# GabrieleCocco/CLFaceDetection

Measured on AMD Instinct MI355X. Metric: candidate windows/sec, 1080p, haarcascade_frontalface_alt, higher is better.
Workload: dtype u32 gathers + f32 stage sums; 1 GPU; BASELINE config 3: 64x1920x1080 8-bit frames per step in the whole job (noise/smooth/blocks mix; sharded by whole frames over 1 GPU), haarcascade_frontalface_alt, scaleFactor 1.1f, raw candidates, frames resident in HBM; frames_on_rank_0=64, windows_per_frame=6290352, parallelism=single GPU, device=AMD Radeon Graphics (gfx950:sramecc+:xnack-), 256 CUs, pipeline=vj_stream, two batches in flight

## Files before the change

clfacedetection_amd/csrc/vj_env.cpp:

```cpp
#include "vj_internal.hpp"
#include "vj_device.hpp"

#include <hip/hip_runtime_api.h>

#include <algorithm>
#include <climits>
#include <cmath>
#include <cstdint>
#include <cstdio>
#include <cstdlib>
#include <cstring>
#include <map>
#include <memory>
#include <string>
#include <tuple>

#include "vj_env_internal.hpp"

using namespace vj;

namespace vj {

static uint32_t f2u(float f) {
    uint32_t u;
// ... 743 lines not shown
        HIP_TRY(hipStreamSynchronize(e->stream));
        if (e->stream2) HIP_TRY(hipStreamSynchronize(e->stream2));
        while ((int)e->plans.size() >= std::max(2, e->plan_cache_max)) {
            auto lru = e->plans.begin();
            for (auto i = e->plans.begin(); i != e->plans.end(); ++i)
                if (i->second->last_used < lru->second->last_used) lru = i;
            lru->second->release_device();
            e->plans.erase(lru);
        }
    }
    auto pl = std::make_unique<Plan>();
    TileThresholds th{e->tile_min_windows, e->tile_accept_windows, e->tile_max_dwords_per_window};
    if (small == 2) th = TileThresholds{64, 64, 8000};
    else if (small == 1) th = TileThresholds{256, 256, 2000};
    else if (small == 3) th = TileThresholds{std::min(384, th.min_windows), std::min(384, th.accept_windows), th.max_dwords_per_window};
    int rc = build_plan(e, *c, W, H, p, pl.get(), split, th, one_pass);
    if (rc) {
        pl->release_device();
        return rc;
    }
    pl->last_used = ++e->plan_tick;
    *out = pl.get();
    e->plans[key] = std::move(pl);
    return VJ_OK;
}

int Lane::create() {
    for (auto& x : ev) HIP_TRY(hipEventCreate(&x));
    for (auto& x : pass_ev) HIP_TRY(hipEventCreate(&x));
    for (auto& x : launch_ev) HIP_TRY(hipEventCreate(&x));
    HIP_TRY(hipEventCreateWithFlags(&upload_done, hipEventDisableTiming));
    HIP_TRY(hipEventCreateWithFlags(&integral_done, hipEventDisableTiming));
    HIP_TRY(hipEventCreateWithFlags(&done, hipEventDisableTiming));
    h_pinned_bytes = (size_t)1 << 20;
    HIP_TRY(hipHostMalloc(&h_pinned, h_pinned_bytes, hipHostMallocDefault));
    return VJ_OK;
}

void Lane::destroy() {
    for (DevBuf* b : {&d_gray, &d_counts, &d_det}) b->release();
    if (h_pinned) (void)hipHostFree(h_pinned);
    if (h_stage) (void)hipHostFree(h_stage);
    h_pinned = h_stage = nullptr;
    for (auto& x : ev) if (x) (void)hipEventDestroy(x);
    for (auto& x : pass_ev) if (x) (void)hipEventDestroy(x);
    for (auto& x : launch_ev) if (x) (void)hipEventDestroy(x);
    for (hipEvent_t* x : {&upload_done, &integral_done, &done}) if (*x) (void)hipEventDestroy(*x);
}

int ensure_image_buffers(vj_env* e, int W, int H, int frames, bool need_gray, int channels, Lane* lane) {
    if (!lane) lane = &e->lane0;
    const size_t fe = frame_elems_for(W, H);
    const uint32_t n_bands = ((uint32_t)H + BAND_ROWS - 1) / BAND_ROWS;
    const uint32_t band_pitch = ((uint32_t)W + 3u) & ~3u;
    int rc;
    const size_t sum_bytes = fe * 4 * (size_t)frames, sq_bytes = fe * 8 * (size_t)frames;
    const bool grow = sum_bytes > e->d_sum.cap || sq_bytes > e->d_sqsum.cap;
    if ((rc = e->d_sum.ensure(sum_bytes))) return rc;
    if ((rc = e->d_sqsum.ensure(sq_bytes))) return rc;
    (void)grow;
    if (need_gray) {
        const size_t gstride = ((size_t)W * (size_t)channels + 3) & ~(size_t)3;
        if ((rc = lane->d_gray.ensure(gstride * (size_t)H * (size_t)frames))) return rc;
    }
    const size_t band_elems = (size_t)frames * n_bands * band_pitch;
    if ((rc = e->d_band_sum.ensure(band_elems * 4))) return rc;
    if ((rc = e->d_band_sq.ensure(band_elems * 4))) return rc;
    if ((rc = e->d_band_sqp.ensure(band_elems * 8))) return rc;
    return VJ_OK;
}

int enqueue_integral(vj_env* e, const uint8_t* d_gray, size_t frame_bytes, int stride, int W, int H, int frames,
                     int channels) {
    IntegralArgs ia;
    memset(&ia, 0, sizeof(ia));
    ia.channels = (uint32_t)channels;
    ia.gray = d_gray;
    ia.gray_frame_bytes = frame_bytes;
    ia.gray_stride = (uint32_t)stride;
    ia.width = (uint32_t)W;
    ia.height = (uint32_t)H;
    ia.n_frames = (uint32_t)frames;
    ia.n_bands = ((uint32_t)H + BAND_ROWS - 1) / BAND_ROWS;
    ia.band_pitch = ((uint32_t)W + 3u) & ~3u;
    ia.band_sum = (uint32_t*)e->d_band_sum.p;
    ia.band_sq = (uint32_t*)e->d_band_sq.p;
    ia.band_sq_prefix = (uint64_t*)e->d_band_sqp.p;
    ia.sum = (uint32_t*)e->d_sum.p;
    ia.sqsum = (uint64_t*)e->d_sqsum.p;
    ia.frame_elems = frame_elems_for(W, H);
    ia.rows_mode = (uint32_t)e->integral_rows_mode;
    const size_t used = (size_t)(W + 1) * (size_t)(H + 1);
    const bool zeroed = e->slack_w == W && e->slack_h == H && e->slack_frames >= frames && e->slack_sum == e->d_sum.p &&
                        e->slack_sq == e->d_sqsum.p;
    for (int f = 0; f < frames && !zeroed; ++f) {
        HIP_TRY(hipMemsetAsync((uint32_t*)e->d_sum.p + (size_t)f * ia.frame_elems + used, 0,
                               (ia.frame_elems - used) * 4, e->stream));
        HIP_TRY(hipMemsetAsync((uint64_t*)e->d_sqsum.p + (size_t)f * ia.frame_elems + used, 0,
                               (ia.frame_elems - used) * 8, e->stream));
    }
    if (!zeroed) {
        e->slack_w = W;
        e->slack_h = H;
        e->slack_frames = frames;
        e->slack_sum = e->d_sum.p;
        e->slack_sq = e->d_sqsum.p;
    }
    int hrc = launch_integral(ia, e->stream);
    if (hrc) {
        set_error("integral launch failed: %s", hipGetErrorString((hipError_t)hrc));
        return VJ_ERR_HIP;
    }
    return VJ_OK;
}

int enqueue_tilted(vj_env* e, const uint8_t* d_gray, size_t frame_bytes, int stride, int W, int H, int frames, int channels) {
    const uint32_t fe = frame_elems_for(W, H);
    int rc;
    if ((rc = e->d_tilted.ensure((size_t)fe * 4u * (size_t)frames))) return rc;
    HIP_TRY(hipMemsetAsync(e->d_tilted.p, 0, (size_t)fe * 4u * (size_t)frames, e->stream));
    TiltedArgs ta;
    memset(&ta, 0, sizeof(ta));
    ta.gray = d_gray;
    ta.gray_frame_bytes = frame_bytes;
    ta.gray_stride = (uint32_t)stride;
    ta.channels = (uint32_t)channels;
    ta.width = (uint32_t)W;
    ta.height = (uint32_t)H;
    ta.n_frames = (uint32_t)frames;
    ta.frame_elems = fe;
    ta.tilted = (uint32_t*)e->d_tilted.p;
    const size_t n_bands = ((size_t)H + 7u) / 8u;
    if ((rc = e->d_tilt_diag.ensure((size_t)frames * n_bands * 2u * (size_t)(W + H) * 4u))) return rc;
    if ((rc = e->d_tilt_col.ensure((size_t)frames * n_bands * (size_t)(W + 1) * 4u))) return rc;
    const int hrc = launch_tilted_bands(ta, (uint32_t*)e->d_tilt_diag.p, (uint32_t*)e->d_tilt_col.p, e->stream);
    if (hrc) {
        set_error("tilted integral launch failed (width %d): %s", W, hipGetErrorString((hipError_t)hrc));
        return hrc == (int)hipErrorInvalidValue ? VJ_ERR_LIMIT : VJ_ERR_HIP;
    }
    return VJ_OK;
}
// ... 88 lines not shown
                for (int y = 0; y < H; ++y) memcpy(st + (size_t)y * gstride, src + (size_t)y * src_stride, row_bytes);
                src = st;
                src_stride = gstride;
            }
        }
        HIP_TRY(hipMemcpy2DAsync(dst, gstride, src, src_stride, row_bytes, (size_t)H,
                                 frames[i].on_device ? hipMemcpyDeviceToDevice : hipMemcpyHostToDevice, cs));
    }
    *d_ptr = (const uint8_t*)lane->d_gray.p;
    *stride = (int)gstride;
    *frame_bytes = gstride * (size_t)H;
    return VJ_OK;
}

struct RawDet {
    int frame;
    uint32_t slot, x, y;
};

struct CountsLayout {
    static constexpr size_t q_counts = (size_t)MAX_SCALES * Q_PARTS;
    static constexpr size_t stage_off_u32 = MAX_PASSES * q_counts + 2;
    static constexpr size_t roi_off_u32 = stage_off_u32 + (size_t)(1 + VJ_MAX_LAUNCHES) * VJ_MAX_STAGES * 2;
    static constexpr size_t q2_off_u32 = roi_off_u32 + 8 + (size_t)VJ_MAX_STAGES * 2;
    static constexpr size_t bytes = (q2_off_u32 + MAX_PASSES * q_counts) * sizeof(uint32_t);
};

static int enqueue_prepare(vj_env* e, Lane* L, Plan* pl, const vj_image* frames, int nf, int W, int H, bool fixed_queue_layout,
                           hipStream_t copy_stream) {
    int rc;
    const int channels = image_channels(frames[0]);
    if ((rc = ensure_image_buffers(e, W, H, nf, true, channels, L))) return rc;
    uint64_t q_entries = 0;
    if (!fixed_queue_layout) {
        if ((rc = layout_queues(pl, nf, &q_entries))) return rc;
        const size_t n_pass = pl->pass_bounds.size() - 1;
        for (size_t ps = 1; ps < n_pass; ++ps)
            if ((rc = e->d_q[ps].ensure(std::max<uint64_t>(q_entries, 1) * sizeof(QEntry)))) return rc;
    }
    if ((rc = L->d_counts.ensure(CountsLayout::bytes))) return rc;
    if (L->det_cap == 0) {
        L->det_cap = e->det_cap_init;
        if ((rc = L->d_det.ensure((size_t)L->det_cap * sizeof(DetEntry)))) return rc;
    }
    const uint8_t* d_gray;
    size_t gray_frame_bytes;
    int gray_stride;
    if ((rc = stage_frames(e, frames, nf, W, H, &d_gray, &gray_frame_bytes, &gray_stride, L, copy_stream))) return rc;
    if (copy_stream) {
        HIP_TRY(hipEventRecord(L->upload_done, copy_stream));
        HIP_TRY(hipStreamWaitEvent(e->stream, L->upload_done, 0));
    }
    L->src_gray = d_gray;
    L->src_frame_bytes = gray_frame_bytes;
    L->src_stride = gray_stride;
    L->src_channels = channels;
    HIP_TRY(hipEventRecord(L->ev[0], e->stream));
    if ((rc = enqueue_integral(e, d_gray, gray_frame_bytes, gray_stride, W, H, nf, channels))) return rc;
    HIP_TRY(hipEventRecord(L->ev[1], e->stream));
    HIP_TRY(hipEventRecord(L->integral_done, e->stream));
    L->nf = nf;
    return VJ_OK;
}

static int enqueue_cascade(vj_env* e, Lane* L, Plan* pl, int W, int , const vj_params& p) {
    int rc;
    const int nf = L->nf;
    const size_t n_pass = pl->pass_bounds.size() - 1;
    const size_t counts_bytes = CountsLayout::bytes;
    constexpr size_t q_counts = CountsLayout::q_counts;
    uint32_t* d_qcount[MAX_PASSES];
    for (int ps = 0; ps < MAX_PASSES; ++ps) d_qcount[ps] = (uint32_t*)L->d_counts.p + ps * q_counts;
    uint32_t* d_qcount2[MAX_PASSES];
    for (int ps = 0; ps < MAX_PASSES; ++ps) d_qcount2[ps] = (uint32_t*)L->d_counts.p + CountsLayout::q2_off_u32 + ps * q_counts;
    uint32_t* d_det_count = (uint32_t*)L->d_counts.p + MAX_PASSES * q_counts;
    unsigned long long* d_stage_entered = (unsigned long long*)((uint32_t*)L->d_counts.p + CountsLayout::stage_off_u32);
    const bool count = (p.flags & VJ_FLAG_COUNTERS) != 0;
    const int n_blocks = std::max(1, e->n_cu * e->blocks_per_cu);
    {
        HIP_TRY(hipMemsetAsync(L->d_counts.p, 0, counts_bytes, e->stream));
        HIP_TRY(hipEventRecord(L->ev[2], e->stream));
        CascadeArgs ca;
        memset(&ca, 0, sizeof(ca));
        ca.sum = (const uint32_t*)e->d_sum.p;
        ca.sqsum = (const uint64_t*)e->d_sqsum.p;
        ca.table = (const uint32_t*)pl->d_table.p;
        ca.scales = (const ScaleDev*)pl->d_scales.p;
        ca.stages = (const StageDev*)pl->d_stages.p;
        ca.units = (const UnitDev*)pl->d_units.p;
        ca.n_units = (uint32_t)pl->units.size();
        ca.tile_units = (const UnitDev*)pl->d_tile_units.p;
        ca.n_tile_units = (uint32_t)pl->tile_units.size();
        ca.n_frames = (uint32_t)nf;
        ca.n_scales = (uint32_t)pl->scales.size();
        ca.frame_elems = pl->frame_elems;
        ca.sum_bytes = (uint32_t)((uint64_t)pl->frame_elems * 4u * (uint64_t)nf);
        ca.stride = (uint32_t)W + 1u;
        ca.gather_waves = (uint32_t)e->gather_waves_for(nf, pl->general);
        ca.total_waves = (uint32_t)n_blocks * ca.gather_waves;
        ca.det = (DetEntry*)L->d_det.p;
        ca.det_count = d_det_count;
        ca.det_cap = L->det_cap;
        ca.signed_mean = (p.flags & VJ_FLAG_SIGNED_MEAN) ? 1u : 0u;
        ca.stage_entered = d_stage_entered;
        ca.tree_ctr = d_stage_entered;
        ca.n_pass = (uint32_t)n_pass;
        for (size_t ps = 0; ps <= n_pass; ++ps) ca.pass_begin[ps] = pl->pass_bounds[ps];
        for (size_t ps = 1; ps < n_pass; ++ps) {
            ca.q_pass[ps] = (QEntry*)e->d_q[ps].p;
            ca.q_pass_count[ps] = d_qcount[ps];
        }
        ca.tile_end = pl->general ? pl->general_prefix : (uint32_t)e->tile_end;
        ca.tile_min_lanes = (uint32_t)e->tile_min_lanes;
        ca.tile_repack_mask = e->tile_repack_mask;
        ca.tile_sp_begin = (!pl->general && (pl->wave_tail || pl->tree2)) ? (uint32_t)e->tile_sp_begin : 0xffffffffu;
        ca.tree2 = pl->tree2 ? 1u : 0u;
        ca.identity_order = pl->general ? 0u : 1u;
        ca.n_seg = e->tile_segments ? pl->tile_n_seg : 0u;
        for (int k = 0; k < 4; ++k) ca.seg_end[k] = pl->tile_seg_end[k];
        ca.seg_chain = pl->tile_seg_chain;
        ca.sp_blocks = (const SpBlock*)pl->d_sp_blocks.p;
        ca.n_sp_blocks = pl->n_sp_blocks;
        ca.tile_ws_min = pl->wave_tail ? (uint32_t)e->tile_ws_min : 0u;
        ca.tile_ws_max = (uint32_t)std::min(e->tile_ws_max, (int)TILE_WS_MAX_WINDOWS);
        ca.pos_mode = pl->pos_mode;
        ca.pos_tab = (const uint32_t*)pl->d_pos_tab.p;
        ca.gather_pairs = e->pairs_for(nf);
        ca.sp_tail_max = (uint32_t)std::max(0, std::min(e->sp_tail_max, 48));
        ca.max_stage_nodes = pl->max_stage_nodes;
        if (pl->skip_mode && pl->n_skip_units) {
            if ((rc = e->d_skip_bits.ensure((size_t)pl->skip_frame_words * 8u * (size_t)nf))) return rc;
            ca.skip_bits = (unsigned long long*)e->d_skip_bits.p;
            ca.skip_frame_words = pl->skip_frame_words;
            ca.skip_units = (const UnitDev*)pl->d_skip_units.p;
            ca.n_skip_units = pl->n_skip_units;
            ca.skip_segs = (const UnitDev*)pl->d_skip_segs.p;
            ca.n_skip_segs = pl->n_skip_segs;
            const int hrc = launch_skip_bitmap(ca, pl->trees, std::max(1, e->n_cu * 4), e->stream);
            if (hrc) {
                set_error("skip bitmap launch failed: %s", hipGetErrorString((hipError_t)hrc));
                return VJ_ERR_HIP;
            }
        }
        int launches = 0;
        std::vector<vj_launch>& linfo = L->linfo;
        linfo.clear();
        auto begin_launch = [&](int kind, int cls, uint32_t sb, uint32_t se, uint32_t lds, hipStream_t st) -> int {
            if (linfo.size() < VJ_MAX_LAUNCHES) HIP_TRY(hipEventRecord(L->launch_ev[2 * linfo.size()], st));
            vj_launch li;
            memset(&li, 0, sizeof(li));
            li.kind = kind;
            li.lds_class = cls;
            li.stage_begin = (int32_t)sb;
            li.stage_end = (int32_t)se;
            li.lds_bytes = lds;
            for (uint32_t slot = 0; slot < pl->scales.size(); ++slot) {
                const ScaleDev& sd = pl->scales[slot];
                const bool in = kind == VJ_LAUNCH_QUEUE ||
                                (kind == VJ_LAUNCH_TILE && sd.tile_rw && sd.tile_row_end > 0 && (int)pl->scales[pl->tile_lead[slot]].tile_class == cls) ||
                                (kind == VJ_LAUNCH_GRID && sd.tile_row_end < sd.ny);
                if (in && sd.scale_idx < 128) li.scale_mask[sd.scale_idx >> 6] |= 1ull << (sd.scale_idx & 63);
            }
            linfo.push_back(li);
            return VJ_OK;
        };
        auto launch_counters = [&]() -> unsigned long long* {
            return d_stage_entered + std::min<size_t>(linfo.size(), VJ_MAX_LAUNCHES) * VJ_MAX_STAGES;
        };
        auto end_launch = [&](hipStream_t st) -> int {
            if (linfo.size() <= VJ_MAX_LAUNCHES) HIP_TRY(hipEventRecord(L->launch_ev[2 * linfo.size() - 1], st));
            return VJ_OK;
        };
        auto pass_is_last = [&](size_t ps) { return pl->seg_last.empty() ? ps + 1 == n_pass : pl->seg_last[ps] != 0; };
        const bool general_kernel = pl->general && pl->seg_last.empty();
        const bool banded = e->q_band_px > 0 && !pl->unit_groups.empty() && !pl->general && n_pass == 2 && nf >= e->q_band_min_frames &&
                            e->tile_min_lanes == 0 && (uint32_t)e->tile_end > pl->pass_bounds[1];
        if (banded) {
            if ((rc = e->d_run_table.ensure((size_t)nf * pl->units.size() * 8u))) return rc;
            ca.run_table = (uint32_t*)e->d_run_table.p;
        }
        auto queue_args = [&](size_t ps, int set = 0) {
            CascadeArgs qa = ca;
            DevBuf* dq = set ? e->d_q2 : e->d_q;
            uint32_t** qc = set ? d_qcount2 : d_qcount;
            qa.stage_begin = pl->pass_bounds[ps];
            qa.stage_end = pl->pass_bounds[ps + 1];
            const bool last = pass_is_last(ps);
            qa.q_in = (const QEntry*)dq[ps].p;
            qa.q_in_count = qc[ps];
            qa.q_ticket = qc[0] + ps * Q_PARTS;
            qa.q_slices = e->q_slices >= 0 ? (uint32_t)std::max(1, e->q_slices)
                                           : (uint32_t)std::max(1, std::min(16, (nf + (int)Q_PARTS - 1) / (int)Q_PARTS));
            qa.min_chunk = (uint32_t)e->min_chunk;
            qa.wide_tail = (e->wide_tail < 0 ? nf <= 4 : e->wide_tail != 0) ? 1u : 0u;
            qa.q_out = last ? nullptr : (QEntry*)dq[ps + 1].p;
            qa.q_out_count = last ? nullptr : qc[ps + 1];
            if (banded && ps == 1) {
                qa.q_groups = (const UnitDev*)pl->d_unit_groups.p;
                qa.n_q_groups = (uint32_t)pl->unit_groups.size();
            }
            if (!pl->seg_fail.empty() && pl->seg_fail[ps] != 0) {
                qa.q_fail = (QEntry*)dq[pl->seg_fail[ps]].p;
                qa.q_fail_count = qc[pl->seg_fail[ps]];
            }
            return qa;
        };
        if (ca.n_units + ca.n_tile_units > 0) {
            int hrc = 0;
            const uint32_t handover = pl->general ? pl->general_prefix : std::max<uint32_t>(ca.tile_end, pl->pass_bounds[1]);
            size_t first_joint_pass = 1;
            if (e->tile_min_lanes == 0)
                while (first_joint_pass < n_pass && pl->pass_bounds[first_joint_pass] < handover) ++first_joint_pass;
            const bool two_streams = e->concurrent && ca.n_tile_units > 0 && ca.n_units > 0;
            const bool split_sets = two_streams && pl->general && !pl->seg_last.empty() && e->tree_split_queues;
            if (split_sets) {
                for (size_t ps = 1; ps < n_pass; ++ps) {
                    if ((rc = e->d_q2[ps].ensure(e->d_q[ps].cap))) return rc;
                    ca.q_pass[ps] = (QEntry*)e->d_q2[ps].p;
                    ca.q_pass_count[ps] = d_qcount2[ps];
                }
                first_joint_pass = n_pass;
            }
            hipStream_t sB = two_streams ? e->stream2 : e->stream;
            if (two_streams) {
                HIP_TRY(hipEventRecord(e->fork_ev, e->stream));
                HIP_TRY(hipStreamWaitEvent(e->stream2, e->fork_ev, 0));
            }
            HIP_TRY(hipEventRecord(L->pass_ev[0], e->stream));
            auto chain_a = [&]() -> int {
            for (uint32_t ci = 0; ci < TILE_CLASSES && !hrc && ca.n_tile_units > 0; ++ci) {
                const uint32_t cls = TILE_CLASSES - 1u - ci;
                const uint32_t n_cls = pl->class_first[cls + 1] - pl->class_first[cls];
                if (!n_cls) continue;
                CascadeArgs ta = ca;
                ta.tile_units = (const UnitDev*)pl->d_tile_units.p + pl->class_first[cls];
                ta.n_tile_units = n_cls;
                ta.tile_lds_bytes = pl->class_lds[cls];
                ta.tile_ticket = d_qcount[0] + (q_counts - 8u * (cls + 1u));
                const int per_cu = std::max(1, std::min(32 / TILE_WAVES, (int)(160u * 1024u / ta.tile_lds_bytes)));
                const int tb = (int)std::min<uint64_t>((uint64_t)n_cls * (uint64_t)nf, (uint64_t)e->n_cu * (uint64_t)per_cu);
                const uint32_t deepest = std::min<uint32_t>((uint32_t)pl->stages.size(), handover);
                if ((rc = begin_launch(VJ_LAUNCH_TILE, (int)cls, 0, deepest, ta.tile_lds_bytes, e->stream))) return rc;
                ta.stage_entered = launch_counters();
                hrc = launch_cascade_tile_pass(ta, pl->trees, count, std::max(1, tb), e->stream);
                if ((rc = end_launch(e->stream))) return rc;
            }
                return VJ_OK;
            };
            const int b_blocks = two_streams ? std::max(1, e->n_cu * e->concurrent_blocks_per_cu) : n_blocks;
            auto chain_b = [&]() -> int {
            if (!hrc && ca.n_units > 0) {
                CascadeArgs ga = queue_args(0);
                ga.total_waves = (uint32_t)b_blocks * ga.gather_waves;
                if ((rc = begin_launch(VJ_LAUNCH_GRID, 0, ga.stage_begin, ga.stage_end, 0, sB))) return rc;
                ga.stage_entered = launch_counters();
                hrc = launch_cascade_pass(ga, true, pl->trees, n_pass == 1, count, general_kernel && n_pass == 1, b_blocks, sB);
                if ((rc = end_launch(sB))) return rc;
                for (size_t ps = 1; ps < first_joint_pass && !hrc; ++ps) {
                    CascadeArgs qa = queue_args(ps);
                    const int qb = split_sets ? n_blocks : b_blocks;
                    qa.total_waves = (uint32_t)qb * qa.gather_waves;
                    if ((rc = begin_launch(VJ_LAUNCH_QUEUE, 0, qa.stage_begin, qa.stage_end, 0, sB))) return rc;
                    qa.stage_entered = launch_counters();
                    hrc = launch_cascade_pass(qa, false, pl->trees, pass_is_last(ps), count, false, qb, sB);
                    if ((rc = end_launch(sB))) return rc;
                }
            } else {
                first_joint_pass = 1;
            }
                return VJ_OK;
            };
            if (two_streams) {
                if ((rc = chain_b())) return rc;
                if ((rc = chain_a())) return rc;
            } else {
                if ((rc = chain_a())) return rc;
                if ((rc = chain_b())) return rc;
            }
            if (two_streams) {
                HIP_TRY(hipEventRecord(e->join_ev, e->stream2));
                HIP_TRY(hipStreamWaitEvent(e->stream, e->join_ev, 0));
            }
            for (size_t ps = 1; ps < n_pass && ps < VJ_MAX_PASSES && ps <= first_joint_pass; ++ps)
                HIP_TRY(hipEventRecord(L->pass_ev[ps], e->stream));
            for (size_t ps = split_sets ? 1 : first_joint_pass; ps < n_pass && !hrc; ++ps) {
                if (ps > first_joint_pass && ps < VJ_MAX_PASSES) HIP_TRY(hipEventRecord(L->pass_ev[ps], e->stream));
                CascadeArgs qa = queue_args(ps, split_sets ? 1 : 0);
                if ((rc = begin_launch(VJ_LAUNCH_QUEUE, 0, qa.stage_begin, qa.stage_end, 0, e->stream))) return rc;
                qa.stage_entered = launch_counters();
                hrc = launch_cascade_pass(qa, false, pl->trees, pass_is_last(ps), count, general_kernel, n_blocks, e->stream);
                if ((rc = end_launch(e->stream))) return rc;
            }
            if (hrc) {
                set_error("cascade launch failed: %s", hipGetErrorString((hipError_t)hrc));
                return VJ_ERR_HIP;
            }
            launches = (int)n_pass;
        }
        if (n_pass <= VJ_MAX_PASSES && launches) HIP_TRY(hipEventRecord(L->pass_ev[n_pass], e->stream));
        HIP_TRY(hipEventRecord(L->ev[3], e->stream));
        L->launches = launches;
    }
    L->n_pass = n_pass;
    L->count = count;
    HIP_TRY(hipMemcpyAsync(L->h_pinned, L->d_counts.p, counts_bytes, hipMemcpyDeviceToHost, e->stream));
    const size_t room = (L->h_pinned_bytes - ((counts_bytes + 255) & ~(size_t)255)) / sizeof(DetEntry);
    L->det_copied = (uint32_t)std::min<size_t>(room, L->det_cap);
    HIP_TRY(hipMemcpyAsync((char*)L->h_pinned + ((counts_bytes + 255) & ~(size_t)255), L->d_det.p, (size_t)L->det_copied * sizeof(DetEntry),
                           hipMemcpyDeviceToHost, e->stream));
    HIP_TRY(hipEventRecord(L->done, e->stream));
    L->pending = true;
    return VJ_OK;
}

static int finish_batch(vj_env* e, Lane* L, Plan* pl, int f0, int W, int H, const vj_params& p, std::vector<RawDet>* dets,
                        vj_counters* ctr, vj_timing* tm, std::vector<DetEntry>* raw_out = nullptr) {
    int rc;
    constexpr size_t q_counts = CountsLayout::q_counts;
    const size_t counts_bytes = CountsLayout::bytes;
    for (int attempt = 0; attempt < 3; ++attempt) {
        HIP_TRY(hipEventSynchronize(L->done));
        L->pending = false;
        const size_t n_pass = L->n_pass;
        const int launches = L->launches;
        const bool count = L->count;
        const std::vector<vj_launch>& linfo = L->linfo;
        const uint32_t n_det = ((const uint32_t*)L->h_pinned)[MAX_PASSES * q_counts];
        float ms_i = 0, ms_c = 0, ms_t = 0;
        HIP_TRY(hipEventElapsedTime(&ms_i, L->ev[0], L->ev[1]));
        HIP_TRY(hipEventElapsedTime(&ms_c, L->ev[2], L->ev[3]));
        HIP_TRY(hipEventElapsedTime(&ms_t, L->ev[0], L->ev[3]));
        if (n_det > L->det_cap) {
            const uint32_t want = grown_cap(L->det_cap, n_det);
            if ((rc = L->d_det.ensure((size_t)want * sizeof(DetEntry)))) return rc;
            L->det_cap = want;
            if (L->shared_integrals) {
                HIP_TRY(hipEventRecord(L->ev[0], e->stream));
                if ((rc = enqueue_integral(e, L->src_gray, L->src_frame_bytes, L->src_stride, W, H, L->nf, L->src_channels))) return rc;
                HIP_TRY(hipEventRecord(L->ev[1], e->stream));
            }
            if ((rc = enqueue_cascade(e, L, pl, W, H, p))) return rc;
            continue;
        }
        if (attempt == 0) tm->integral_ms += ms_i;
        tm->cascade_ms += ms_c;
        tm->total_ms += ms_t;
        if (launches && n_pass <= VJ_MAX_PASSES)
            for (size_t ps = 0; ps < n_pass; ++ps) {
                float ms = 0;
                HIP_TRY(hipEventElapsedTime(&ms, L->pass_ev[ps], L->pass_ev[ps + 1]));
                tm->pass_ms[ps] += ms;
                tm->pass_stage_begin[ps] = (int32_t)pl->pass_bounds[ps];
                tm->pass_stage_end[ps] = (int32_t)pl->pass_bounds[ps + 1];
            }
        tm->n_cascade_launches = std::max(tm->n_cascade_launches, launches);
        const unsigned long long* se_all = (const unsigned long long*)((const uint32_t*)L->h_pinned + CountsLayout::stage_off_u32);
        if (linfo.size() <= VJ_MAX_LAUNCHES) {
            for (size_t i = 0; i < linfo.size(); ++i) {
                float ms = 0;
                HIP_TRY(hipEventElapsedTime(&ms, L->launch_ev[2 * i], L->launch_ev[2 * i + 1]));
                vj_launch acc = tm->launch[i];
                tm->launch[i] = linfo[i];
                tm->launch[i].ms = acc.ms + ms;
                const unsigned long long* se = se_all + (1 + i) * VJ_MAX_STAGES;
// ... 1274 lines not shown
    if (check_params(*p)) return VJ_ERR_ARG;
    if ((uint64_t)(width + 1) * (uint64_t)(height + 3) >= (1ull << 30)) {
        set_error("image too large");
        return VJ_ERR_LIMIT;
    }
    HIP_TRY(hipSetDevice(e->device));
    auto s = std::make_unique<vj_stream>();
    s->e = e;
    s->p = *p;
    s->W = width;
    s->H = height;
    s->CH = CH;
    s->max_batch = max_batch;
    s->plan = std::make_unique<Plan>();
    struct Guard {
        vj_stream* s;
        ~Guard() { if (s) vj_stream_destroy(s); }
    } guard{nullptr};
    const vj_env::Balance* bal = balance_of(e, c, width, height, *p, max_batch, false);
    TileThresholds sth{e->tile_min_windows, e->tile_accept_windows, e->tile_max_dwords_per_window};
    if (bal && balance_choice(bal, -1).thr == 1 && !e->tile_thresholds_set) sth = TileThresholds{std::min(384, sth.min_windows), std::min(384, sth.accept_windows), sth.max_dwords_per_window};
    int rc = build_plan(e, *c, width, height, *p, s->plan.get(), bal ? bal->best : e->split_for(max_batch, *p), sth);
    if (rc) {
        s->plan->release_device();
        return rc;
    }
    vj_stream* raw = s.release();
    guard.s = raw;
    if ((uint64_t)max_batch > max_frames_per_subbatch(e, raw->plan.get())) {
        set_error("max_batch %d exceeds what one launch sequence can address at this frame size (%llu frames)", max_batch,
                  (unsigned long long)max_frames_per_subbatch(e, raw->plan.get()));
        return VJ_ERR_LIMIT;
    }
    for (Lane& L : raw->lanes) {
        if ((rc = L.create())) return rc;
        L.shared_integrals = true;
    }
    HIP_TRY(hipStreamCreateWithFlags(&raw->copy, hipStreamNonBlocking));
    for (Lane& L : raw->lanes)
        if ((rc = ensure_image_buffers(e, width, height, max_batch, true, CH, &L))) return rc;
    uint64_t q_entries = 0;
    if ((rc = layout_queues(raw->plan.get(), max_batch, &q_entries))) return rc;
    const size_t n_pass = raw->plan->pass_bounds.size() - 1;
    for (size_t ps = 1; ps < n_pass; ++ps)
        if ((rc = e->d_q[ps].ensure(std::max<uint64_t>(q_entries, 1) * sizeof(QEntry)))) return rc;
    guard.s = nullptr;
    *out = raw;
    return VJ_OK;
}

int vj_stream_submit(vj_stream* s, const vj_image* frames, int n_frames) {
    if (!s || !frames || n_frames <= 0 || n_frames > s->max_batch) return VJ_ERR_ARG;
    if (s->n_pending >= 2) {
        set_error("two batches are pending: collect one before submitting the next");
        return VJ_ERR_LIMIT;
    }
    int W, H, CH;
    int rc = check_frames(frames, n_frames, &W, &H, &CH);
    if (rc) return rc;
    if (W != s->W || H != s->H || CH != s->CH) {
        set_error("frames do not have the stream's size / channel count");
        return VJ_ERR_ARG;
    }
    vj_env* e = s->e;
    HIP_TRY(hipSetDevice(e->device));
    const int lane = s->n_pending == 0 ? 0 : 1 - s->fifo[0];
    Lane* L = &s->lanes[lane];
    HIP_TRY(hipEventSynchronize(L->integral_done));
    if ((rc = enqueue_prepare(e, L, s->plan.get(), frames, n_frames, W, H, true, s->copy))) return rc;
    if ((rc = enqueue_cascade(e, L, s->plan.get(), W, H, s->p))) return rc;
    s->fifo[s->n_pending] = lane;
    s->n_frames_of[lane] = n_frames;
    s->n_pending++;
    return VJ_OK;
}

int vj_stream_collect(vj_stream* s, vj_result* out) {
    if (!s || !out) return VJ_ERR_ARG;
// ... 40 lines not shown
```

clfacedetection_amd/csrc/vj_env_internal.hpp:

```cpp
#pragma once
#include "vj_internal.hpp"
#include "vj_device.hpp"

#include <hip/hip_runtime_api.h>

#include <algorithm>
#include <cstring>
#include <map>
#include <memory>
#include <tuple>
#include <vector>

namespace vj {

#define HIP_TRY(expr)                                                                        \
    do {                                                                                     \
        hipError_t e_ = (expr);                                                              \
        if (e_ != hipSuccess) {                                                              \
            set_error("%s failed: %s (%s:%d)", #expr, hipGetErrorString(e_), __FILE__, __LINE__); \
            return VJ_ERR_HIP;                                                               \
        }                                                                                    \
    } while (0)

struct DevBuf {
// ... 63 lines not shown
    float tile_split = 0.0f;
    void release_device() {
        for (DevBuf* b : {&d_table, &d_scales, &d_stages, &d_units, &d_tile_units, &d_sp_blocks, &d_skip_units, &d_skip_segs, &d_pos_tab, &d_unit_groups}) b->release();
    }
};

struct CvPlan {
    std::vector<CvScaleDev> scales;
    StageProgram prog;
    uint32_t n_stages = 0, n_order = 0, n_rows = 0;
    bool trees = false, is_tree = false, has_tilted = false, tree2 = false;
    DevBuf d_table, d_scales, d_stages, d_rows;
    uint32_t n_tile_scales = 0, n_rows_rest = 0, bits_frame_words = 0, n_bit_segs = 0;
    int row_blocks = 1;
    uint32_t tree_prefix = 0;
    CvChainDev chains = {};
    bool prune = false;
    DevBuf d_prune;
    int tq_shift = -1;
    uint64_t tile_windows = 0;
    int tq_split_frames = 0;
    uint32_t class_first[3] = {0, 0, 0}, class_lds[2] = {0, 0};
    DevBuf d_tiles, d_rows_rest, d_bit_segs;
    uint64_t last_used = 0;
    void release_device() {
        for (DevBuf* b : {&d_table, &d_scales, &d_stages, &d_rows, &d_tiles, &d_rows_rest, &d_bit_segs, &d_prune}) b->release();
    }
};

}

namespace vj {


struct Lane {
    DevBuf d_gray, d_counts, d_det;
    uint32_t det_cap = 0;
    void* h_pinned = nullptr;
    size_t h_pinned_bytes = 0;
    void* h_stage = nullptr;
    size_t h_stage_bytes = 0;
    hipEvent_t ev[4] = {};
    hipEvent_t pass_ev[VJ_MAX_PASSES + 1] = {};
    hipEvent_t launch_ev[2 * VJ_MAX_LAUNCHES] = {};
    hipEvent_t upload_done = nullptr, integral_done = nullptr, done = nullptr;
    bool pending = false;
    int nf = 0, first_frame = 0;
    const uint8_t* src_gray = nullptr;
    size_t src_frame_bytes = 0;
    int src_stride = 0, src_channels = 1;
    bool shared_integrals = false;
    size_t n_pass = 0;
    int launches = 0;
    bool count = false;
    uint32_t det_copied = 0;
    std::vector<vj_launch> linfo;
    int create();
    void destroy();
};

}

namespace vj {

struct Tunables {
    int max_subbatch = 0;
    uint32_t det_cap_init = 1u << 16;
    int concurrent = 1;
    int gather_waves = -1;
    int gather_waves_for(int n_frames, bool general) const {
        if (general) return vj::WAVES_PER_BLOCK;
        const int w = gather_waves > 0 ? gather_waves : (n_frames >= 8 ? vj::GATHER_WAVES_MAX : vj::WAVES_PER_BLOCK);
        return std::min(std::max(w, 1), (int)vj::GATHER_WAVES_MAX);
    }
    int concurrent_blocks_per_cu = 1;
    float tile_split = 1.5f;
    float tile_split_mid = 1.75f;
    float tile_split_small = 0.0f;
// ... 29 lines not shown
    int tile_ws_max = 512;
    int tile_ws_min = 48;
    int group_max = (int)vj::GROUP_MAX;
    bool tree_split_queues = true;
    bool cv_tiles = true;
    int cv_tile_ws_max = 512;
    int cv_row_blocks = -1;
    int cv_row_blocks_tree = 2, cv_tile_min_windows_tree = 256;
    int cv_tail_max = 64;
    int cv_tree_chunk = 64, cv_tree_chain_blocks = 2;
    bool cv_tiles_tilted = true;
    bool cv_tree2 = true;
    int cv_row_band_px = 128;
    bool cv_tree_chains = true;
    int cv_tree_queue_cap = 0;
    int cv_tile_min_windows0 = 2048;
    int cv_tile_min_windows = -1;
    bool rois_on_device = true;
    int wide_tail = -1;
    int min_chunk = 32;
    int q_band_px = 128;
    int q_group_units = 4;
    int q_band_min_frames = 8;
    int q_slices = -1;
    int sp_tail_max = 48;
    int gather_pairs = -1;
    uint32_t pairs_for(int n_frames) const { return gather_pairs >= 0 ? (uint32_t)gather_pairs : n_frames <= 4 ? 2u : 0u; }
    std::vector<int> split_override;
    std::vector<int> pass_cut_nodes{35};
};

}

struct vj_env : vj::Tunables {
    int device = 0;
    int tile_group = 4;
    hipStream_t stream = nullptr;
    vj::Lane lane0;
    hipEvent_t fork_ev = nullptr, join_ev = nullptr;
    hipStream_t stream2 = nullptr;
    char name[256] = "";
    int n_cu = 0;
    vj::DevBuf d_sum, d_sqsum, d_band_sum, d_band_sq, d_band_sqp;
    vj::DevBuf d_tilted;
    vj::DevBuf d_tilt_diag, d_tilt_col;
    vj::DevBuf d_out;
    int slack_w = 0, slack_h = 0, slack_frames = 0;
    void *slack_sum = nullptr, *slack_sq = nullptr;
    vj::DevBuf d_q[vj::MAX_PASSES];
    vj::DevBuf d_q2[vj::MAX_PASSES];
    vj::DevBuf d_skip_bits;
    vj::DevBuf d_run_table;
    vj::DevBuf d_rois, d_roi_units, d_roi_det, d_roi_tiles;
    uint32_t roi_tile_cap = 0;
    vj::DevBuf d_group;
    uint32_t roi_unit_cap = 0, roi_det_cap = 0;
    typedef std::tuple<uint64_t, int, int, int, int, int, int, uint32_t, uint64_t, uint64_t, uint32_t, uint32_t> PlanKey;
    std::map<PlanKey, std::unique_ptr<vj::Plan>> plans;
    struct Balance {
        float cur = 0, best = 0, best_ms = 0, cand_ms = 0;
        int phase = 0;
        int samples = 0, moved = 0, calls = 0;
        int thr = 0;
        bool thr_tried = false, far_tried = false;
        int n_ref = 0;
        int off_ref = 0;
        bool first_slow = false;
        uint64_t last_used = 0;
        uint32_t calls_total = 0, calls_on_candidate = 0;
    };
    typedef std::tuple<PlanKey, int> BalanceKey;
    std::map<BalanceKey, Balance> balance;
    uint64_t balance_tick = 0;
    typedef std::tuple<uint64_t, int, int, int, int, uint64_t, int> CvPlanKey;
    std::map<CvPlanKey, std::unique_ptr<vj::CvPlan>> cv_plans;
    vj::DevBuf d_cv_det, d_cv_counts;
    vj::DevBuf d_cv_accept, d_cv_tq;
    vj::DevBuf d_cv_fail_rows, d_cv_fail_walk;
    vj::DevBuf d_canny_cls, d_canny_label, d_canny_flag, d_edges, d_edge_sum, d_cv_prune_bits;
    int edge_slack_w = 0, edge_slack_h = 0, edge_slack_frames = 0;
    void* edge_slack_sum = nullptr;
    uint64_t plan_tick = 0;
    int cv_tq_shift = 4;
};

namespace vj {
int image_channels(const vj_image& im);
int check_single_image(const vj_image* image, int* ch_out);
uint32_t frame_elems_for(int W, int H);
int ensure_image_buffers(vj_env* e, int W, int H, int frames, bool need_gray, int channels = 1, Lane* lane = nullptr);
int enqueue_integral(vj_env* e, const uint8_t* d_gray, size_t frame_bytes, int stride, int W, int H, int frames,
                     int channels = 1);
int stage_frames(vj_env* e, const vj_image* frames, int n, int W, int H, const uint8_t** d_ptr, size_t* frame_bytes,
                 int* stride, Lane* lane = nullptr, hipStream_t copy_stream = nullptr);
int enqueue_tilted(vj_env* e, const uint8_t* d_gray, size_t frame_bytes, int stride, int W, int H, int frames, int channels);
}
```

Baseline: 10.33 billion windows/s.

## Give each stream lane private integral buffers and overlap prep/readback on aux stream

Each lane of the stream pipeline now owns its own set of integral, band, queue, skip-bitmap and run-table buffers. Upload, integral, counts memset and skip-bitmap work run on the lane's auxiliary copy stream, and readback is deferred onto that stream. The aim is to let one batch's integral and prep overlap another batch's cascade instead of serialising on shared buffers and the main stream. This costs extra HBM per lane, adds more cross-stream event dependencies, and falls back to shared buffers on allocation failure or when VJ_STREAM_SERIAL is set.

```diff
diff --git a/clfacedetection_amd/csrc/vj_env.cpp b/clfacedetection_amd/csrc/vj_env.cpp
--- a/clfacedetection_amd/csrc/vj_env.cpp
+++ b/clfacedetection_amd/csrc/vj_env.cpp
@@ -799,6 +799,9 @@
     HIP_TRY(hipEventCreateWithFlags(&upload_done, hipEventDisableTiming));
     HIP_TRY(hipEventCreateWithFlags(&integral_done, hipEventDisableTiming));
     HIP_TRY(hipEventCreateWithFlags(&done, hipEventDisableTiming));
+    HIP_TRY(hipEventCreateWithFlags(&ready, hipEventDisableTiming));
+    for (auto& x : chain_end) HIP_TRY(hipEventCreateWithFlags(&x, hipEventDisableTiming));
+    HIP_TRY(hipEventCreate(&chain_b_start));
     h_pinned_bytes = (size_t)1 << 20;
     HIP_TRY(hipHostMalloc(&h_pinned, h_pinned_bytes, hipHostMallocDefault));
     return VJ_OK;
@@ -806,39 +809,42 @@
 
 void Lane::destroy() {
     for (DevBuf* b : {&d_gray, &d_counts, &d_det}) b->release();
+    if (own) own->release_set();
+    own.reset();
     if (h_pinned) (void)hipHostFree(h_pinned);
     if (h_stage) (void)hipHostFree(h_stage);
     h_pinned = h_stage = nullptr;
     for (auto& x : ev) if (x) (void)hipEventDestroy(x);
     for (auto& x : pass_ev) if (x) (void)hipEventDestroy(x);
     for (auto& x : launch_ev) if (x) (void)hipEventDestroy(x);
-    for (hipEvent_t* x : {&upload_done, &integral_done, &done}) if (*x) (void)hipEventDestroy(*x);
+    for (hipEvent_t* x : {&upload_done, &integral_done, &done, &ready, &chain_end[0], &chain_end[1], &chain_b_start}) if (*x) (void)hipEventDestroy(*x);
 }
 
 int ensure_image_buffers(vj_env* e, int W, int H, int frames, bool need_gray, int channels, Lane* lane) {
     if (!lane) lane = &e->lane0;
+    DevSet* ds = lane->own ? lane->own.get() : e;
     const size_t fe = frame_elems_for(W, H);
     const uint32_t n_bands = ((uint32_t)H + BAND_ROWS - 1) / BAND_ROWS;
     const uint32_t band_pitch = ((uint32_t)W + 3u) & ~3u;
     int rc;
     const size_t sum_bytes = fe * 4 * (size_t)frames, sq_bytes = fe * 8 * (size_t)frames;
-    const bool grow = sum_bytes > e->d_sum.cap || sq_bytes > e->d_sqsum.cap;
-    if ((rc = e->d_sum.ensure(sum_bytes))) return rc;
-    if ((rc = e->d_sqsum.ensure(sq_bytes))) return rc;
-    (void)grow;
+    if ((rc = ds->d_sum.ensure(sum_bytes))) return rc;
+    if ((rc = ds->d_sqsum.ensure(sq_bytes))) return rc;
     if (need_gray) {
         const size_t gstride = ((size_t)W * (size_t)channels + 3) & ~(size_t)3;
         if ((rc = lane->d_gray.ensure(gstride * (size_t)H * (size_t)frames))) return rc;
     }
     const size_t band_elems = (size_t)frames * n_bands * band_pitch;
-    if ((rc = e->d_band_sum.ensure(band_elems * 4))) return rc;
-    if ((rc = e->d_band_sq.ensure(band_elems * 4))) return rc;
-    if ((rc = e->d_band_sqp.ensure(band_elems * 8))) return rc;
+    if ((rc = ds->d_band_sum.ensure(band_elems * 4))) return rc;
+    if ((rc = ds->d_band_sq.ensure(band_elems * 4))) return rc;
+    if ((rc = ds->d_band_sqp.ensure(band_elems * 8))) return rc;
     return VJ_OK;
 }
 
 int enqueue_integral(vj_env* e, const uint8_t* d_gray, size_t frame_bytes, int stride, int W, int H, int frames,
-                     int channels) {
+                     int channels, DevSet* set, hipStream_t stream) {
+    DevSet* ds = set ? set : e;
+    hipStream_t st = stream ? stream : e->stream;
     IntegralArgs ia;
     memset(&ia, 0, sizeof(ia));
     ia.channels = (uint32_t)channels;
@@ -850,30 +856,30 @@
     ia.n_frames = (uint32_t)frames;
     ia.n_bands = ((uint32_t)H + BAND_ROWS - 1) / BAND_ROWS;
     ia.band_pitch = ((uint32_t)W + 3u) & ~3u;
-    ia.band_sum = (uint32_t*)e->d_band_sum.p;
-    ia.band_sq = (uint32_t*)e->d_band_sq.p;
-    ia.band_sq_prefix = (uint64_t*)e->d_band_sqp.p;
-    ia.sum = (uint32_t*)e->d_sum.p;
-    ia.sqsum = (uint64_t*)e->d_sqsum.p;
+    ia.band_sum = (uint32_t*)ds->d_band_sum.p;
+    ia.band_sq = (uint32_t*)ds->d_band_sq.p;
+    ia.band_sq_prefix = (uint64_t*)ds->d_band_sqp.p;
+    ia.sum = (uint32_t*)ds->d_sum.p;
+    ia.sqsum = (uint64_t*)ds->d_sqsum.p;
     ia.frame_elems = frame_elems_for(W, H);
     ia.rows_mode = (uint32_t)e->integral_rows_mode;
     const size_t used = (size_t)(W + 1) * (size_t)(H + 1);
-    const bool zeroed = e->slack_w == W && e->slack_h == H && e->slack_frames >= frames && e->slack_sum == e->d_sum.p &&
-                        e->slack_sq == e->d_sqsum.p;
+    const bool zeroed = ds->slack_w == W && ds->slack_h == H && ds->slack_frames >= frames && ds->slack_sum == ds->d_sum.p &&
+                        ds->slack_sq == ds->d_sqsum.p;
     for (int f = 0; f < frames && !zeroed; ++f) {
-        HIP_TRY(hipMemsetAsync((uint32_t*)e->d_sum.p + (size_t)f * ia.frame_elems + used, 0,
-                               (ia.frame_elems - used) * 4, e->stream));
-        HIP_TRY(hipMemsetAsync((uint64_t*)e->d_sqsum.p + (size_t)f * ia.frame_elems + used, 0,
-                               (ia.frame_elems - used) * 8, e->stream));
+        HIP_TRY(hipMemsetAsync((uint32_t*)ds->d_sum.p + (size_t)f * ia.frame_elems + used, 0,
+                               (ia.frame_elems - used) * 4, st));
+        HIP_TRY(hipMemsetAsync((uint64_t*)ds->d_sqsum.p + (size_t)f * ia.frame_elems + used, 0,
+                               (ia.frame_elems - used) * 8, st));
     }
     if (!zeroed) {
-        e->slack_w = W;
-        e->slack_h = H;
-        e->slack_frames = frames;
-        e->slack_sum = e->d_sum.p;
-        e->slack_sq = e->d_sqsum.p;
-    }
-    int hrc = launch_integral(ia, e->stream);
+        ds->slack_w = W;
+        ds->slack_h = H;
+        ds->slack_frames = frames;
+        ds->slack_sum = ds->d_sum.p;
+        ds->slack_sq = ds->d_sqsum.p;
+    }
+    int hrc = launch_integral(ia, st);
     if (hrc) {
         set_error("integral launch failed: %s", hipGetErrorString((hipError_t)hrc));
         return VJ_ERR_HIP;
@@ -1028,11 +1034,13 @@
     const int channels = image_channels(frames[0]);
     if ((rc = ensure_image_buffers(e, W, H, nf, true, channels, L))) return rc;
     uint64_t q_entries = 0;
+    DevSet* ds = L->own ? L->own.get() : e;
+    hipStream_t si = L->own ? L->aux : e->stream;
     if (!fixed_queue_layout) {
         if ((rc = layout_queues(pl, nf, &q_entries))) return rc;
         const size_t n_pass = pl->pass_bounds.size() - 1;
         for (size_t ps = 1; ps < n_pass; ++ps)
-            if ((rc = e->d_q[ps].ensure(std::max<uint64_t>(q_entries, 1) * sizeof(QEntry)))) return rc;
+            if ((rc = ds->d_q[ps].ensure(std::max<uint64_t>(q_entries, 1) * sizeof(QEntry)))) return rc;
     }
     if ((rc = L->d_counts.ensure(CountsLayout::bytes))) return rc;
     if (L->det_cap == 0) {
@@ -1045,17 +1053,38 @@
     if ((rc = stage_frames(e, frames, nf, W, H, &d_gray, &gray_frame_bytes, &gray_stride, L, copy_stream))) return rc;
     if (copy_stream) {
         HIP_TRY(hipEventRecord(L->upload_done, copy_stream));
-        HIP_TRY(hipStreamWaitEvent(e->stream, L->upload_done, 0));
+        if (si != copy_stream) HIP_TRY(hipStreamWaitEvent(si, L->upload_done, 0));
     }
     L->src_gray = d_gray;
     L->src_frame_bytes = gray_frame_bytes;
     L->src_stride = gray_stride;
     L->src_channels = channels;
-    HIP_TRY(hipEventRecord(L->ev[0], e->stream));
-    if ((rc = enqueue_integral(e, d_gray, gray_frame_bytes, gray_stride, W, H, nf, channels))) return rc;
-    HIP_TRY(hipEventRecord(L->ev[1], e->stream));
-    HIP_TRY(hipEventRecord(L->integral_done, e->stream));
+    HIP_TRY(hipEventRecord(L->ev[0], si));
+    if ((rc = enqueue_integral(e, d_gray, gray_frame_bytes, gray_stride, W, H, nf, channels, ds, si))) return rc;
+    HIP_TRY(hipEventRecord(L->ev[1], si));
+    HIP_TRY(hipEventRecord(L->integral_done, si));
     L->nf = nf;
+    return VJ_OK;
+}
+
+static int enqueue_readback(vj_env* e, Lane* L) {
+    const size_t counts_bytes = CountsLayout::bytes;
+    hipStream_t sr = e->stream;
+    if (L->overlapped()) {
+        sr = L->aux;
+        HIP_TRY(hipStreamWaitEvent(sr, L->chain_end[0], 0));
+        if (L->two_chains) HIP_TRY(hipStreamWaitEvent(sr, L->chain_end[1], 0));
+        if (L->late_pass_ev && L->launches && L->n_pass <= VJ_MAX_PASSES)
+            for (size_t ps = 1; ps <= L->n_pass; ++ps) HIP_TRY(hipEventRecord(L->pass_ev[ps], sr));
+        HIP_TRY(hipEventRecord(L->ev[3], sr));
+    }
+    HIP_TRY(hipMemcpyAsync(L->h_pinned, L->d_counts.p, counts_bytes, hipMemcpyDeviceToHost, sr));
+    const size_t room = (L->h_pinned_bytes - ((counts_bytes + 255) & ~(size_t)255)) / sizeof(DetEntry);
+    L->det_copied = (uint32_t)std::min<size_t>(room, L->det_cap);
+    HIP_TRY(hipMemcpyAsync((char*)L->h_pinned + ((counts_bytes + 255) & ~(size_t)255), L->d_det.p, (size_t)L->det_copied * sizeof(DetEntry),
+                           hipMemcpyDeviceToHost, sr));
+    HIP_TRY(hipEventRecord(L->done, sr));
+    L->readback_queued = true;
     return VJ_OK;
 }
 
@@ -1073,13 +1102,18 @@
     unsigned long long* d_stage_entered = (unsigned long long*)((uint32_t*)L->d_counts.p + CountsLayout::stage_off_u32);
     const bool count = (p.flags & VJ_FLAG_COUNTERS) != 0;
     const int n_blocks = std::max(1, e->n_cu * e->blocks_per_cu);
+    DevSet* ds = L->own ? L->own.get() : e;
+    const bool ov = L->overlapped();
+    hipStream_t s0 = ov ? L->aux : e->stream;
+    L->two_chains = L->late_pass_ev = L->readback_queued = false;
     {
-        HIP_TRY(hipMemsetAsync(L->d_counts.p, 0, counts_bytes, e->stream));
-        HIP_TRY(hipEventRecord(L->ev[2], e->stream));
+        HIP_TRY(hipMemsetAsync(L->d_counts.p, 0, counts_bytes, s0));
+        bool ev2_set = !ov;
+        if (!ov) HIP_TRY(hipEventRecord(L->ev[2], e->stream));
         CascadeArgs ca;
         memset(&ca, 0, sizeof(ca));
-        ca.sum = (const uint32_t*)e->d_sum.p;
-        ca.sqsum = (const uint64_t*)e->d_sqsum.p;
+        ca.sum = (const uint32_t*)ds->d_sum.p;
+        ca.sqsum = (const uint64_t*)ds->d_sqsum.p;
         ca.table = (const uint32_t*)pl->d_table.p;
         ca.scales = (const ScaleDev*)pl->d_scales.p;
         ca.stages = (const StageDev*)pl->d_stages.p;
@@ -1103,7 +1137,7 @@
         ca.n_pass = (uint32_t)n_pass;
         for (size_t ps = 0; ps <= n_pass; ++ps) ca.pass_begin[ps] = pl->pass_bounds[ps];
         for (size_t ps = 1; ps < n_pass; ++ps) {
-            ca.q_pass[ps] = (QEntry*)e->d_q[ps].p;
+            ca.q_pass[ps] = (QEntry*)ds->d_q[ps].p;
             ca.q_pass_count[ps] = d_qcount[ps];
         }
         ca.tile_end = pl->general ? pl->general_prefix : (uint32_t)e->tile_end;
@@ -1125,18 +1159,25 @@
         ca.sp_tail_max = (uint32_t)std::max(0, std::min(e->sp_tail_max, 48));
         ca.max_stage_nodes = pl->max_stage_nodes;
         if (pl->skip_mode && pl->n_skip_units) {
-            if ((rc = e->d_skip_bits.ensure((size_t)pl->skip_frame_words * 8u * (size_t)nf))) return rc;
-            ca.skip_bits = (unsigned long long*)e->d_skip_bits.p;
+            if ((rc = ds->d_skip_bits.ensure((size_t)pl->skip_frame_words * 8u * (size_t)nf))) return rc;
+            ca.skip_bits = (unsigned long long*)ds->d_skip_bits.p;
             ca.skip_frame_words = pl->skip_frame_words;
             ca.skip_units = (const UnitDev*)pl->d_skip_units.p;
             ca.n_skip_units = pl->n_skip_units;
             ca.skip_segs = (const UnitDev*)pl->d_skip_segs.p;
             ca.n_skip_segs = pl->n_skip_segs;
-            const int hrc = launch_skip_bitmap(ca, pl->trees, std::max(1, e->n_cu * 4), e->stream);
+            if (!ev2_set) HIP_TRY(hipEventRecord(L->ev[2], s0));
+            ev2_set = true;
+            const int hrc = launch_skip_bitmap(ca, pl->trees, std::max(1, e->n_cu * 4), s0);
             if (hrc) {
                 set_error("skip bitmap launch failed: %s", hipGetErrorString((hipError_t)hrc));
                 return VJ_ERR_HIP;
             }
+        }
+        if (ov) {
+            HIP_TRY(hipEventRecord(L->ready, s0));
+            HIP_TRY(hipStreamWaitEvent(e->stream, L->ready, 0));
+            if (!ev2_set) HIP_TRY(hipEventRecord(L->ev[2], e->stream));
         }
         int launches = 0;
         std::vector<vj_launch>& linfo = L->linfo;
@@ -1172,12 +1213,12 @@
         const bool banded = e->q_band_px > 0 && !pl->unit_groups.empty() && !pl->general && n_pass == 2 && nf >= e->q_band_min_frames &&
                             e->tile_min_lanes == 0 && (uint32_t)e->tile_end > pl->pass_bounds[1];
         if (banded) {
-            if ((rc = e->d_run_table.ensure((size_t)nf * pl->units.size() * 8u))) return rc;
-            ca.run_table = (uint32_t*)e->d_run_table.p;
+            if ((rc = ds->d_run_table.ensure((size_t)nf * pl->units.size() * 8u))) return rc;
+            ca.run_table = (uint32_t*)ds->d_run_table.p;
         }
         auto queue_args = [&](size_t ps, int set = 0) {
             CascadeArgs qa = ca;
-            DevBuf* dq = set ? e->d_q2 : e->d_q;
+            DevBuf* dq = set ? ds->d_q2 : ds->d_q;
             uint32_t** qc = set ? d_qcount2 : d_qcount;
             qa.stage_begin = pl->pass_bounds[ps];
             qa.stage_end = pl->pass_bounds[ps + 1];
@@ -1211,14 +1252,18 @@
             const bool split_sets = two_streams && pl->general && !pl->seg_last.empty() && e->tree_split_queues;
             if (split_sets) {
                 for (size_t ps = 1; ps < n_pass; ++ps) {
-                    if ((rc = e->d_q2[ps].ensure(e->d_q[ps].cap))) return rc;
-                    ca.q_pass[ps] = (QEntry*)e->d_q2[ps].p;
+                    if ((rc = ds->d_q2[ps].ensure(ds->d_q[ps].cap))) return rc;
+                    ca.q_pass[ps] = (QEntry*)ds->d_q2[ps].p;
                     ca.q_pass_count[ps] = d_qcount2[ps];
                 }
                 first_joint_pass = n_pass;
             }
             hipStream_t sB = two_streams ? e->stream2 : e->stream;
-            if (two_streams) {
+            if (two_streams && ov) {
+                HIP_TRY(hipStreamWaitEvent(e->stream2, L->ready, 0));
+                HIP_TRY(hipEventRecord(L->chain_b_start, e->stream2));
+                L->two_chains = true;
+            } else if (two_streams) {
                 HIP_TRY(hipEventRecord(e->fork_ev, e->stream));
                 HIP_TRY(hipStreamWaitEvent(e->stream2, e->fork_ev, 0));
             }
@@ -1273,11 +1318,13 @@
                 if ((rc = chain_a())) return rc;
                 if ((rc = chain_b())) return rc;
             }
-            if (two_streams) {
+            if (L->two_chains) HIP_TRY(hipEventRecord(L->chain_end[1], e->stream2));
+            L->late_pass_ev = L->two_chains && !split_sets && first_joint_pass >= n_pass;
+            if (two_streams && !L->late_pass_ev) {
                 HIP_TRY(hipEventRecord(e->join_ev, e->stream2));
                 HIP_TRY(hipStreamWaitEvent(e->stream, e->join_ev, 0));
             }
-            for (size_t ps = 1; ps < n_pass && ps < VJ_MAX_PASSES && ps <= first_joint_pass; ++ps)
+            for (size_t ps = 1; ps < n_pass && ps < VJ_MAX_PASSES && ps <= first_joint_pass && !L->late_pass_ev; ++ps)
                 HIP_TRY(hipEventRecord(L->pass_ev[ps], e->stream));
             for (size_t ps = split_sets ? 1 : first_joint_pass; ps < n_pass && !hrc; ++ps) {
                 if (ps > first_joint_pass && ps < VJ_MAX_PASSES) HIP_TRY(hipEventRecord(L->pass_ev[ps], e->stream));
@@ -1293,18 +1340,14 @@
             }
             launches = (int)n_pass;
         }
-        if (n_pass <= VJ_MAX_PASSES && launches) HIP_TRY(hipEventRecord(L->pass_ev[n_pass], e->stream));
-        HIP_TRY(hipEventRecord(L->ev[3], e->stream));
+        if (n_pass <= VJ_MAX_PASSES && launches && !L->late_pass_ev) HIP_TRY(hipEventRecord(L->pass_ev[n_pass], e->stream));
+        if (ov) HIP_TRY(hipEventRecord(L->chain_end[0], e->stream));
+        else HIP_TRY(hipEventRecord(L->ev[3], e->stream));
         L->launches = launches;
     }
     L->n_pass = n_pass;
     L->count = count;
-    HIP_TRY(hipMemcpyAsync(L->h_pinned, L->d_counts.p, counts_bytes, hipMemcpyDeviceToHost, e->stream));
-    const size_t room = (L->h_pinned_bytes - ((counts_bytes + 255) & ~(size_t)255)) / sizeof(DetEntry);
-    L->det_copied = (uint32_t)std::min<size_t>(room, L->det_cap);
-    HIP_TRY(hipMemcpyAsync((char*)L->h_pinned + ((counts_bytes + 255) & ~(size_t)255), L->d_det.p, (size_t)L->det_copied * sizeof(DetEntry),
-                           hipMemcpyDeviceToHost, e->stream));
-    HIP_TRY(hipEventRecord(L->done, e->stream));
+    if (!ov && (rc = enqueue_readback(e, L))) return rc;
     L->pending = true;
     return VJ_OK;
 }
@@ -1315,6 +1358,7 @@
     constexpr size_t q_counts = CountsLayout::q_counts;
     const size_t counts_bytes = CountsLayout::bytes;
     for (int attempt = 0; attempt < 3; ++attempt) {
+        if (!L->readback_queued && (rc = enqueue_readback(e, L))) return rc;
         HIP_TRY(hipEventSynchronize(L->done));
         L->pending = false;
         const size_t n_pass = L->n_pass;
@@ -1326,6 +1370,12 @@
         HIP_TRY(hipEventElapsedTime(&ms_i, L->ev[0], L->ev[1]));
         HIP_TRY(hipEventElapsedTime(&ms_c, L->ev[2], L->ev[3]));
         HIP_TRY(hipEventElapsedTime(&ms_t, L->ev[0], L->ev[3]));
+        if (L->overlapped()) {
+            float lead = 0;
+            if (L->two_chains) HIP_TRY(hipEventElapsedTime(&lead, L->chain_b_start, L->ev[2]));
+            ms_c += std::max(lead, 0.0f);
+            ms_t = ms_i + ms_c;
+        }
         if (n_det > L->det_cap) {
             const uint32_t want = grown_cap(L->det_cap, n_det);
             if ((rc = L->d_det.ensure((size_t)want * sizeof(DetEntry)))) return rc;
@@ -2666,18 +2716,47 @@
                   (unsigned long long)max_frames_per_subbatch(e, raw->plan.get()));
         return VJ_ERR_LIMIT;
     }
+    for (Lane& L : raw->lanes)
+        if ((rc = L.create())) return rc;
+    HIP_TRY(hipStreamCreateWithFlags(&raw->copy, hipStreamNonBlocking));
+    uint64_t q_entries = 0;
+    if ((rc = layout_queues(raw->plan.get(), max_batch, &q_entries))) return rc;
+    const Plan* pl = raw->plan.get();
+    const size_t n_pass = pl->pass_bounds.size() - 1;
+    const char* serial_env = getenv("VJ_STREAM_SERIAL");
+    bool own_sets = !(serial_env && atoi(serial_env) != 0);
+    auto fill_set = [&](Lane& L) -> int {
+        int r;
+        if ((r = ensure_image_buffers(e, width, height, max_batch, false, CH, &L))) return r;
+        DevSet* ds = L.own.get();
+        for (size_t ps = 1; ps < n_pass; ++ps) {
+            if ((r = ds->d_q[ps].ensure(std::max<uint64_t>(q_entries, 1) * sizeof(QEntry)))) return r;
+            if (pl->general && !pl->seg_last.empty() && (r = ds->d_q2[ps].ensure(ds->d_q[ps].cap))) return r;
+        }
+        if (!pl->unit_groups.empty() && (r = ds->d_run_table.ensure((size_t)max_batch * pl->units.size() * 8u))) return r;
+        if (pl->skip_mode && pl->n_skip_units && (r = ds->d_skip_bits.ensure((size_t)pl->skip_frame_words * 8u * (size_t)max_batch))) return r;
+        return VJ_OK;
+    };
     for (Lane& L : raw->lanes) {
-        if ((rc = L.create())) return rc;
-        L.shared_integrals = true;
-    }
-    HIP_TRY(hipStreamCreateWithFlags(&raw->copy, hipStreamNonBlocking));
+        if (!own_sets) break;
+        L.own = std::make_unique<DevSet>();
+        L.aux = raw->copy;
+        rc = fill_set(L);
+        if (rc == VJ_ERR_NOMEM) own_sets = false;
+        else if (rc) return rc;
+    }
+    if (!own_sets) {
+        for (Lane& L : raw->lanes) {
+            if (L.own) L.own->release_set();
+            L.own.reset();
+            L.aux = nullptr;
+            L.shared_integrals = true;
+        }
+        for (size_t ps = 1; ps < n_pass; ++ps)
+            if ((rc = e->d_q[ps].ensure(std::max<uint64_t>(q_entries, 1) * sizeof(QEntry)))) return rc;
+    }
     for (Lane& L : raw->lanes)
         if ((rc = ensure_image_buffers(e, width, height, max_batch, true, CH, &L))) return rc;
-    uint64_t q_entries = 0;
-    if ((rc = layout_queues(raw->plan.get(), max_batch, &q_entries))) return rc;
-    const size_t n_pass = raw->plan->pass_bounds.size() - 1;
-    for (size_t ps = 1; ps < n_pass; ++ps)
-        if ((rc = e->d_q[ps].ensure(std::max<uint64_t>(q_entries, 1) * sizeof(QEntry)))) return rc;
     guard.s = nullptr;
     *out = raw;
     return VJ_OK;
diff --git a/clfacedetection_amd/csrc/vj_env_internal.hpp b/clfacedetection_amd/csrc/vj_env_internal.hpp
--- a/clfacedetection_amd/csrc/vj_env_internal.hpp
+++ b/clfacedetection_amd/csrc/vj_env_internal.hpp
@@ -119,6 +119,23 @@
 
 namespace vj {
 
+struct DevSet {
+    DevBuf d_sum, d_sqsum, d_band_sum, d_band_sq, d_band_sqp;
+    int slack_w = 0, slack_h = 0, slack_frames = 0;
+    void *slack_sum = nullptr, *slack_sq = nullptr;
+    DevBuf d_q[MAX_PASSES];
+    DevBuf d_q2[MAX_PASSES];
+    DevBuf d_skip_bits;
+    DevBuf d_run_table;
+    void release_set() {
+        for (DevBuf* b : {&d_sum, &d_sqsum, &d_band_sum, &d_band_sq, &d_band_sqp, &d_skip_bits, &d_run_table}) b->release();
+        for (DevBuf& b : d_q) b.release();
+        for (DevBuf& b : d_q2) b.release();
+        slack_w = slack_h = slack_frames = 0;
+        slack_sum = slack_sq = nullptr;
+    }
+};
+
 
 struct Lane {
     DevBuf d_gray, d_counts, d_det;
@@ -131,6 +148,13 @@
     hipEvent_t pass_ev[VJ_MAX_PASSES + 1] = {};
     hipEvent_t launch_ev[2 * VJ_MAX_LAUNCHES] = {};
     hipEvent_t upload_done = nullptr, integral_done = nullptr, done = nullptr;
+    std::unique_ptr<DevSet> own;
+    hipStream_t aux = nullptr;
+    hipEvent_t ready = nullptr, chain_end[2] = {}, chain_b_start = nullptr;
+    bool two_chains = false;
+    bool late_pass_ev = false;
+    bool readback_queued = false;
+    bool overlapped() const { return own != nullptr; }
     bool pending = false;
     int nf = 0, first_frame = 0;
     const uint8_t* src_gray = nullptr;
@@ -226,7 +250,7 @@
 
 }
 
-struct vj_env : vj::Tunables {
+struct vj_env : vj::Tunables, vj::DevSet {
     int device = 0;
     int tile_group = 4;
     hipStream_t stream = nullptr;
@@ -235,16 +259,9 @@
     hipStream_t stream2 = nullptr;
     char name[256] = "";
     int n_cu = 0;
-    vj::DevBuf d_sum, d_sqsum, d_band_sum, d_band_sq, d_band_sqp;
     vj::DevBuf d_tilted;
     vj::DevBuf d_tilt_diag, d_tilt_col;
     vj::DevBuf d_out;
-    int slack_w = 0, slack_h = 0, slack_frames = 0;
-    void *slack_sum = nullptr, *slack_sq = nullptr;
-    vj::DevBuf d_q[vj::MAX_PASSES];
-    vj::DevBuf d_q2[vj::MAX_PASSES];
-    vj::DevBuf d_skip_bits;
-    vj::DevBuf d_run_table;
     vj::DevBuf d_rois, d_roi_units, d_roi_det, d_roi_tiles;
     uint32_t roi_tile_cap = 0;
     vj::DevBuf d_group;
@@ -284,7 +301,7 @@
 uint32_t frame_elems_for(int W, int H);
 int ensure_image_buffers(vj_env* e, int W, int H, int frames, bool need_gray, int channels = 1, Lane* lane = nullptr);
 int enqueue_integral(vj_env* e, const uint8_t* d_gray, size_t frame_bytes, int stride, int W, int H, int frames,
-                     int channels = 1);
+                     int channels = 1, DevSet* set = nullptr, hipStream_t stream = nullptr);
 int stage_frames(vj_env* e, const vj_image* frames, int n, int W, int H, const uint8_t** d_ptr, size_t* frame_bytes,
                  int* stride, Lane* lane = nullptr, hipStream_t copy_stream = nullptr);
 int enqueue_tilted(vj_env* e, const uint8_t* d_gray, size_t frame_bytes, int stride, int W, int H, int frames, int channels);
```

After: 10.17 billion windows/s. 0.984x the previous value.
